# bababyVN/medical-image-segmentation-and-classification

Measured on AMD Instinct MI355X. Metric: images/sec (train step) Attention U-Net 256x256 bs=32/GPU, higher is better.
Workload: dtype bf16; 1 GPU; AttentionUNet 256x256 train step (fwd+BCE+bwd+clip+AdamW), bs=32/GPU, NHWC bf16 activations, fp32 master weights; global_batch=32, parallelism=dp1, hip_graph=False, wgrad_side_stream=True, plan_replay=C (mi355_plan_run)

## Files before the change

include/mi355conv.h:

```cpp
#ifndef MI355CONV_H_
#define MI355CONV_H_

#include <stdint.h>

#ifdef __cplusplus
extern "C" {
#endif

typedef struct ihipStream_t* mi355_stream_t;

enum { MI355_F32 = 0, MI355_BF16 = 1, MI355_F16 = 2 };
enum { MI355_OK = 0, MI355_ERR_ARG = -1, MI355_ERR_UNSUPPORTED = -2, MI355_ERR_RUNTIME = -3 };

int mi355_version(void);
const char* mi355_last_error(void);


int mi355_pack_input_nchw(const float* x, void* y, int N, int C, int H, int W, int Cpad, int dtype,
                          mi355_stream_t s);
int mi355_pack_input_im2col3(const float* x, void* y, int N, int C, int H, int W, int dtype, mi355_stream_t s);
int mi355_unpack_output_nchw(const void* x, float* y, int N, int C, int H, int W, int ld, int dtype,
                             mi355_stream_t s);
int mi355_pack_nchw(const float* x, void* y, int N, int C, int H, int W, int ld, int dtype, mi355_stream_t s);

int mi355_pack_conv_weight(const float* w, void* wf, void* wb, int Co, int Ci, int Cip, int KH, int KW,
                           int transposed, int dtype, mi355_stream_t s);

int mi355_pack_conv_weights_batched(const int64_t* table, int n, int fields ,
                                    int dtype, mi355_stream_t s);

int mi355_conv2d_igemm(const void* in, const void* wk, const float* bias, void* out,
                       int N, int Hi, int Wi, int Ci, int ldi,
                       int Ho, int Wo, int Co, int ldo,
                       int KH, int KW, int mul, int kmul, int off, int div, int up,
                       int accumulate, float* stats, int dtype, mi355_stream_t s);
int mi355_conv2d_igemm_variant(int Hi, int Wi, int Ci, int Ho, int Wo, int Co, int KH, int KW, int mul, int kmul, int off,
                               int div, int up, int dtype);
int mi355_conv2d_igemm_variant_n(int N, int Hi, int Wi, int Ci, int Ho, int Wo, int Co, int KH, int KW, int mul, int kmul,
                                 int off, int div, int up, int dtype);
int mi355_conv2d_igemm_dma_tile(int N, int Ho, int Wo, int Ci, int Co);
int mi355_conv2d_igemm_generic_tile(int N, int Ho, int Wo, int Co);
int mi355_conv2d_igemm_stat_rows(int N, int Hi, int Wi, int Ci, int Ho, int Wo, int Co, int KH, int KW,
                                 int mul, int kmul, int off, int div, int up, int dtype);
int mi355_conv2d_igemm_pool2_ok(int N, int Hi, int Wi, int Ci, int Ho, int Wo, int Co, int KH, int KW,
                                int mul, int kmul, int off, int div, int up, int dtype);
const char* mi355_conv2d_igemm_kernel_name(int N, int Hi, int Wi, int Ci, int Ho, int Wo, int Co, int KH, int KW,
                                           int mul, int kmul, int off, int div, int up, int dtype);

int mi355_conv2d_wgrad_splits(int N, int Ho, int Wo, int Ci, int Co, int KH, int KW);
int mi355_conv2d_wgrad_variant(int N, int Ho, int Wo, int KH, int KW, int stride, int pad, int dtype);
const char* mi355_conv2d_wgrad_kernel_name(int N, int Ho, int Wo, int Ci, int Co, int KH, int KW, int stride, int pad, int dtype);
int mi355_conv2d_wgrad(const void* x, const void* dy, float* ws, int splits,
                       int N, int Hi, int Wi, int Ci, int ldx,
                       int Ho, int Wo, int Co, int ldy,
                       int KH, int KW, int stride, int pad, int up, int dtype, mi355_stream_t s);
int mi355_conv2d_wgrad_multi_ok(int N, int Ho, int Wo, int dtype);
int mi355_conv2d_wgrad_multi(const void* x0, const void* dy0, const void* x1, const void* dy1, const void* x2, const void* dy2,
                             const void* x3, const void* dy3, const void* x4, const void* dy4, const void* x5, const void* dy5,
                             int napp, float* ws, int splits, int N, int Hi, int Wi, int Ci, int ldx, int Ho, int Wo, int Co,
                             int ldy, int up, int dtype, mi355_stream_t s);
int mi355_conv2d_wgrad_reduce(const float* ws, int splits, float* dw, int Co, int Ci, int Ci_real,
                              int KH, int KW, int transposed, float beta, mi355_stream_t s);


int mi355_rowreduce_blocks(long long M);
int mi355_bn_stats(const void* x, float* partial, long long M, int C, int ld, int dtype, mi355_stream_t s);
int mi355_bn_finalize(const float* partial, int nblocks, long long M, int C, const float* gamma,
                      const float* beta, float* running_mean, float* running_var, int64_t* nbt,
                      float momentum, float eps, float* scale, float* shift, float* mean, float* invstd,
                      mi355_stream_t s);
int mi355_fold_rows(const float* partial, int rows, int rowlen, float* out, int nsplit, mi355_stream_t s);
int mi355_bn_fold_bias(const float* bias, const float* scale, const float* shift, float* out, int C, mi355_stream_t s);
int mi355_bn_eval_coeffs(const float* gamma, const float* beta, const float* running_mean,
                         const float* running_var, float eps, int C, float* scale, float* shift,
                         mi355_stream_t s);
int mi355_bn_act(const void* x, int ldx, const float* scale, const float* shift,
                 const void* x2, int ldx2, const float* scale2, const float* shift2,
                 const void* res, int ldr, void* y, int ldy, long long M, int C, int act, int dtype,
                 mi355_stream_t s);
int mi355_bn_act_pool2(const void* x, int ldx, const float* scale, const float* shift, void* y, int ldy, void* p, int ldp,
                       int N, int H, int W, int C, int act, int dtype, mi355_stream_t s);
int mi355_bn_act_windows(const void* x, int ldx, const float* scale, const float* shift, const void* res, int ldr, void* y, int ldy,
                         int N, int H, int W, int C, int act, int dtype, mi355_stream_t s);
int mi355_bn_bwd_reduce_rows(long long M);
int mi355_bn_bwd_reduce(const void* dy, int lddy, const void* y, int ldy, const void* x, int ldx,
                        const float* mean, const float* invstd, const float* mscale, const float* mshift,
                        float* partial, long long M, int C, int act, int dtype, mi355_stream_t s);
int mi355_bn_bwd_finalize(const float* partial, int nblocks, int C, float* sums, float* dgamma, float* dbeta,
                          float acc, mi355_stream_t s);
int mi355_bn_bwd_finalize_at(const float* partial, int nblocks, int nq, int q0, int q1, int C, float* sums, float* dgamma,
                             float* dbeta, float acc, mi355_stream_t s);
int mi355_bn_bwd_apply(const void* dy, int lddy, const void* y, int ldy, const void* x, int ldx,
                       const float* gamma, const float* mean, const float* invstd, const float* mscale,
                       const float* mshift, const float* sums, void* dx, int lddx, void* dres, int lddres,
                       void* dpost, int lddpost, int post_acc, float* dbias_partial,
                       long long M, int C, int act, int dtype, mi355_stream_t s);
int mi355_bn_bwd_apply_post4(const void* dy, int lddy, const void* y, int ldy, const void* x, int ldx,
                             const float* gamma, const float* mean, const float* invstd, const float* mscale,
                             const float* mshift, const float* sums, void* dx, int lddx, void* dpost, int lddpost,
                             int post_acc, const void* ex0, const void* ex1, const void* ex2, const void* ex3, int ldex,
                             long long M, int C, int act, int dtype, mi355_stream_t s);
int mi355_bn_bwd_pool2_ok(int H, int W, int C, int dtype);
int mi355_bn_bwd_reduce_pool2_rows(long long M);
int mi355_bn_bwd_reduce_pool2(const void* dy, int lddy, const void* dp, int lddp, const void* x, int ldx, const float* mean,
                              const float* invstd, const float* mscale, const float* mshift, float* partial,
                              int N, int H, int W, int C, int dtype, mi355_stream_t s);
int mi355_bn_bwd_apply_pool2(const void* dy, int lddy, const void* dp, int lddp, const void* x, int ldx, const float* gamma,
                             const float* mean, const float* invstd, const float* mscale, const float* mshift,
                             const float* sums, void* dx, int lddx, int N, int H, int W, int C, int dtype, mi355_stream_t s);
int mi355_colsum_finalize(const float* partial, int nblocks, int stride, int C, float* out, float acc,
                          mi355_stream_t s);
int mi355_colsum(const void* x, int ld, float* partial, long long M, int C, int dtype, mi355_stream_t s);

int mi355_maxpool_fwd(const void* x, int ldx, void* y, int ldy, int N, int H, int W, int C,
                      int k, int stride, int pad, int dtype, mi355_stream_t s);
int mi355_maxpool_bwd(const void* x, int ldx, const void* dy, int lddy, void* dx, int lddx,
                      int N, int H, int W, int C, int k, int stride, int pad, int accumulate, int dtype,
                      mi355_stream_t s);
int mi355_upsample2_bwd(const void* dy, int lddy, void* dx, int lddx, int N, int H, int W, int C,
                        int accumulate, int dtype, mi355_stream_t s);
int mi355_add(const void* a, int lda, const void* b, int ldb, void* y, int ldy, long long M, int C, int dtype,
              mi355_stream_t s);
int mi355_relu_fwd(const void* x, int ldx, void* y, int ldy, long long M, int C, int dtype, mi355_stream_t s);
int mi355_relu_bwd(const void* dy, int lddy, const void* y, int ldy, void* dx, int lddx, long long M, int C,
                   int dtype, mi355_stream_t s);

int mi355_rowdot_fwd(const void* x, int ldx, const float* w, const float* b, float* z, float* partial,
                     long long M, int C, int HW, int K, int dtype, mi355_stream_t s);
int mi355_rowdot_bwd(const float* dz, const void* x, int ldx, const float* w, void* dx, int lddx,
                     float* partial, long long M, int C, int relu_mask, int HW, int K, int accumulate, int dtype,
                     mi355_stream_t s);
int mi355_gate_mul_fwd(const void* x, int ldx, const float* z, const float* scale, const float* shift,
                       void* y, int ldy, long long M, int C, int dtype, mi355_stream_t s);
int mi355_gate_mul_bwd(const void* dy, int lddy, const void* x, int ldx, const float* z, const float* scale,
                       const float* shift, const float* mean, const float* invstd, void* dx, int lddx,
                       int accumulate, float* dzn, float* partial, long long M, int C, int dtype,
                       mi355_stream_t s);
int mi355_bn1_bwd_apply(const float* dzn, const float* z, const float* gamma, const float* mean,
                        const float* invstd, const float* sums, float* dz, long long M, mi355_stream_t s);
int mi355_gate_psi_fwd_ok(int C, int dtype);
int mi355_gate_psi_fwd(const void* g1, int ldg, const void* x1, int ldx, const float* scale_g, const float* shift_g,
                       const float* scale_x, const float* shift_x, const float* w, const float* b, float* z,
                       float* partial, long long M, int C, int dtype, mi355_stream_t s);
int mi355_gate_bn_bwd_reduce_rows(long long M);
int mi355_gate_bn_bwd_reduce(const float* dz, const void* g1, int ldg, const void* x1, int ldx, const float* scale_g,
                             const float* shift_g, const float* mean_g, const float* invstd_g, const float* scale_x,
                             const float* shift_x, const float* mean_x, const float* invstd_x, const float* w,
                             float* partial, long long M, int C, int dtype, mi355_stream_t s);
int mi355_gate_bn_bwd_apply(const float* dz, const void* g1, int ldg, const void* x1, int ldx, const float* scale_g,
                            const float* shift_g, const float* mean_g, const float* invstd_g, const float* scale_x,
                            const float* shift_x, const float* mean_x, const float* invstd_x, const float* w,
                            const float* gamma_g, const float* gamma_x, const float* sums_g, const float* sums_x,
                            void* dg1, int lddg, void* dx1, int lddx, long long M, int C, int dtype, mi355_stream_t s);

int mi355_global_pool_fwd(const void* x, int ldx, float* y, int32_t* argmax, int N, int HW, int C, int is_max,
                          int dtype, mi355_stream_t s);
int mi355_global_pool_bwd(const float* dy, const int32_t* argmax, void* dx, int lddx, int N, int HW, int C,
                          int is_max, int dtype, mi355_stream_t s);
int mi355_linear_fwd(const float* x, const float* w, const float* bias, float* y, int B, int I, int O, int relu,
                     mi355_stream_t s);
int mi355_linear_bwd(const float* x, const float* w, const float* y, const float* dy, float* dx, float* dw,
                     float* db, int B, int I, int O, int relu, float beta, float* scratch, mi355_stream_t s);
int mi355_linear_bwd_scratch(int B, int I, int O);
int mi355_dropout_fwd(const float* x, float* y, uint8_t* mask, long long n, float p, uint64_t seed,
                      const int32_t* counter, mi355_stream_t s);
int mi355_dropout_bwd(const float* dy, const uint8_t* mask, float* dx, long long n, float p, mi355_stream_t s);

int mi355_bce_logits(const float* z, const float* t, float* loss, float* dz, const float* gscale, long long n,
                     mi355_stream_t s);
int mi355_ce_smooth(const float* z, const int64_t* y, float* loss, float* dz, const float* gscale, int B,
                    int C, float smoothing, mi355_stream_t s);
int mi355_ce_mix(const float* z, const int64_t* ya, const int64_t* yb, const float* lam, const float* weight, float* loss,
                 float* dz, const float* gscale, int B, int C, float smoothing, mi355_stream_t s);
int mi355_seg_loss_rows(int B, long long per);
int mi355_seg_loss_fwd(const float* z, const float* t, int B, long long per, float bce_weight, float dice_weight,
                       float smooth, int per_sample, float* partial, float* state, float* loss, mi355_stream_t s);
int mi355_seg_loss_bwd(const float* z, const float* t, int B, long long per, float bce_weight, const float* state,
                       const float* gscale, float* dz, mi355_stream_t s);
int mi355_sdist_ws_ints(int B, int H, int W);
int mi355_signed_dist2(const float* target, int B, int H, int W, float thr, int32_t* ws, long long ws_ints,
                       int32_t* sd2, mi355_stream_t s);
int mi355_boundary_loss_rows(int B, long long per);
int mi355_boundary_loss_fwd(const float* z, const int32_t* sd2, int B, long long per, float weight, const float* base,
                            float* partial, float* loss, mi355_stream_t s);
int mi355_boundary_loss_bwd(const float* z, const int32_t* sd2, int B, long long per, float weight, const float* gscale,
                            int accumulate, float* dz, mi355_stream_t s);
int mi355_segsort_tile(void);
int mi355_segsort_ws_ints(int S, long long len);
int mi355_segsort_f32(const float* keys, int S, long long len, int32_t* ws, long long ws_ints, int32_t* perm,
                      mi355_stream_t s);
int mi355_lovasz_ws_ints(int S, long long len);
int mi355_lovasz_fwd(const float* z, const float* t, int S, long long len, float thr, float weight, const float* base,
                     int32_t* ws, long long ws_ints, float* coef, float* loss, mi355_stream_t s);
int mi355_lovasz_bwd(const float* coef, long long n, const float* gscale, int accumulate, float* dz, mi355_stream_t s);
int mi355_rank_ws_ints(int S, long long len);
// ... 121 lines not shown
```

medical-image-segmentation-and-classification_amd/csrc/conv_gemm256.hpp:

```cpp
#pragma once
#include "common.hpp"

struct Gemm256Cfg {
  static constexpr int BM = 256, BN = 128, BK = 64, NS = 3;
  static constexpr int A_BYTES = BM * BK * 2, B_BYTES = BN * BK * 2, STAGE = A_BYTES + B_BYTES;
  static constexpr int C_PITCH = BN * 2 + 16;
  static constexpr int LDS_BYTES = NS * STAGE;
  static_assert(BM * C_PITCH + 4 * 2 * BN * 4 <= LDS_BYTES, "the C tile and the statistics scratch go on top of the dead ring");
};

template <typename T>
__global__ __launch_bounds__(512, 2) void conv_gemm256_kernel(const ConvArgs a, const int mode) {
  static_assert(sizeof(T) == 2, "bf16 / fp16 only");
  typedef Gemm256Cfg Cfg;
  constexpr int BM = Cfg::BM, BN = Cfg::BN, BK = Cfg::BK, NS = Cfg::NS, EPC = 8;
  constexpr int A_BYTES = Cfg::A_BYTES, STAGE = Cfg::STAGE, C_PITCH = Cfg::C_PITCH;
  constexpr int A_IT = BM / 8 / 8, B_IT = BN / 8 / 8, PER_TILE = A_IT + B_IT;
  extern __shared__ __attribute__((aligned(16))) unsigned char lds[];

  const int tid = threadIdx.x, lane = tid & 63, wave = __builtin_amdgcn_readfirstlane(tid >> 6);
  const int l16 = lane & 15, c4 = lane >> 4;
  const int wm = wave >> 1, wn = wave & 1;
  const int taps = a.KH * a.KW;
  const int NCOL = mode == 1 ? taps * a.Co : a.Co;
  const int NT = NCOL / BN;
  const int bid = xcd_tile(blockIdx.x, gridDim.x);
  const int mt = bid / NT, nt = bid - mt * NT;
  const int m0 = mt * BM, n0 = nt * BN;
  const int ptap = mode == 1 ? n0 / a.Co : 0, co0 = mode == 1 ? n0 - ptap * a.Co : n0;
  const T* __restrict__ in = reinterpret_cast<const T*>(a.in);
  const T* __restrict__ wk = reinterpret_cast<const T*>(a.wk);
  auto fsw = [](int row) { return (row >> 1) & 7; };

  const int lrow = lane >> 3, slot = lane & 7;
  const T* a_src[A_IT];
#pragma unroll
  for (int i = 0; i < A_IT; ++i) {
    const int row = (wave + 8 * i) * 8 + lrow;
    const int m = m0 + row;
    long long pix;
    if (mode == 1) {
      pix = m;
    } else {
      const int n = m / a.HoWo, rem = m - n * a.HoWo;
      const int ho = rem / a.Wo, wo = rem - ho * a.Wo;
      pix = ((long long)n * a.Hi + ho * a.mul) * a.Wi + wo * a.mul;
    }
    a_src[i] = in + pix * a.ldi + (slot ^ fsw(row)) * EPC;
  }
  const T* b_src[B_IT];
#pragma unroll
  for (int i = 0; i < B_IT; ++i) {
    const int row = (wave + 8 * i) * 8 + lrow;
    b_src[i] = wk + ((size_t)(co0 + row) * taps + ptap) * a.Ci + (slot ^ fsw(row)) * EPC;
  }
  const unsigned lds0 = lds_addr(lds);
  const int KC = a.Ci / BK;
  const int KT = (mode == 1 ? 1 : taps) * KC;
  int i_tap = 0, i_c0 = 0, i_stage = 0;
  size_t i_aoff = 0, i_boff = 0;
  auto issue_piece = [&](int j) __attribute__((always_inline)) {
    const unsigned st = lds0 + i_stage * STAGE;
    if (j < A_IT) dma16(a_src[j] + i_aoff, st + (wave + 8 * j) * 1024);
    else dma16(b_src[j - A_IT] + i_boff, st + A_BYTES + (wave + 8 * (j - A_IT)) * 1024);
  };
  auto issue_advance = [&]() __attribute__((always_inline)) {
    i_c0 += BK;
    if (i_c0 == a.Ci) {
      i_c0 = 0;
      ++i_tap;
    }
    const int kh = i_tap / a.KW, kw = i_tap - kh * a.KW;
    i_aoff = (mode == 1 ? (size_t)0 : ((size_t)kh * a.Wi + kw) * a.ldi) + i_c0;
    i_boff = (mode == 1 ? (size_t)0 : (size_t)i_tap * a.Ci) + i_c0;
    i_stage = i_stage + 1 == NS ? 0 : i_stage + 1;
  };

  f32x4 acc[4][4];
#pragma unroll
  for (int cb = 0; cb < 4; ++cb)
#pragma unroll
    for (int pb = 0; pb < 4; ++pb) acc[cb][pb] = f32x4{0.f, 0.f, 0.f, 0.f};

  int fa_w[4], fa_p[4];
#pragma unroll
  for (int b = 0; b < 4; ++b) {
    const int rw = wn * 64 + b * 16 + l16, rp = wm * 64 + b * 16 + l16;
    fa_w[b] = A_BYTES + rw * 128 + fsw(rw) * 16;
    fa_p[b] = rp * 128 + fsw(rp) * 16;
  }
  auto frag = [&](const unsigned char* st, int base, int kh2) __attribute__((always_inline)) {
    return *reinterpret_cast<const bf16x8*>(st + (base ^ ((kh2 * 4 + c4) << 4)));
  };

  int issued = 0;
#pragma unroll
  for (int t = 0; t < NS - 1; ++t) {
    if (issued < KT) {
#pragma unroll
      for (int j = 0; j < PER_TILE; ++j) issue_piece(j);
      issue_advance();
      ++issued;
    }
  }

  int stage = 0;
  for (int kt = 0; kt < KT; ++kt) {
    if (kt + 1 < KT) wait_vmcnt<PER_TILE>(); else wait_vmcnt<0>();
    __builtin_amdgcn_s_barrier();
    const unsigned char* st = lds + stage * STAGE;
    const bool more = issued < KT;
    bf16x8 w0[4], p0[4], w1[4], p1[4];
#pragma unroll
    for (int b = 0; b < 4; ++b) {
      w0[b] = frag(st, fa_w[b], 0);
      p0[b] = frag(st, fa_p[b], 0);
    }
#pragma unroll
    for (int b = 0; b < 4; ++b) {
      w1[b] = frag(st, fa_w[b], 1);
      p1[b] = frag(st, fa_p[b], 1);
    }
#pragma unroll
    for (int cb = 0; cb < 4; ++cb) {
#pragma unroll
      for (int pb = 0; pb < 4; ++pb) acc[cb][pb] = mfma_16x16x32<T>(w0[cb], p0[pb], acc[cb][pb]);
      if (more) {
        issue_piece(cb);
      }
    }
#pragma unroll
    for (int cb = 0; cb < 4; ++cb) {
#pragma unroll
      for (int pb = 0; pb < 4; ++pb) acc[cb][pb] = mfma_16x16x32<T>(w1[cb], p1[pb], acc[cb][pb]);
      if (more && cb < PER_TILE - 4) issue_piece(4 + cb);
    }
    if (more) {
      issue_advance();
      ++issued;
    }
    stage = stage + 1 == NS ? 0 : stage + 1;
  }
  __syncthreads();

  T* __restrict__ out = reinterpret_cast<T*>(a.out);
  unsigned char* const cst = lds;
  float* const red = reinterpret_cast<float*>(lds + BM * C_PITCH);
  struct alignas(8) Pack4 { T v[4]; };
#pragma unroll
  for (int cb = 0; cb < 4; ++cb) {
    const int ch = wn * 64 + cb * 16 + 4 * c4;
    const f32x4 bias4 = a.bias ? *reinterpret_cast<const f32x4*>(a.bias + co0 + ch) : f32x4{0.f, 0.f, 0.f, 0.f};
    f32x4 sm = {0.f, 0.f, 0.f, 0.f}, sq = {0.f, 0.f, 0.f, 0.f};
#pragma unroll
    for (int pb = 0; pb < 4; ++pb) {
      const int row = wm * 64 + pb * 16 + l16;
      Pack4 pk;
#pragma unroll
      for (int r = 0; r < 4; ++r) {
        const float v = acc[cb][pb][r] + bias4[r];
        pk.v[r] = from_f32<T>(a.relu ? fmaxf(v, 0.f) : v);
        const float q = to_f32<T>(pk.v[r]);
        sm[r] += q;
        sq[r] += q * q;
      }
      *reinterpret_cast<Pack4*>(cst + row * C_PITCH + ch * 2) = pk;
    }
    if (a.stats) {
#pragma unroll
      for (int r = 0; r < 4; ++r) {
        const float s1 = row16_sum(sm[r]), s2 = row16_sum(sq[r]);
        if (l16 == 0) {
          red[(wm * 2 + 0) * BN + ch + r] = s1;
          red[(wm * 2 + 1) * BN + ch + r] = s2;
        }
      }
    }
  }
  __syncthreads();
  if (a.stats && tid < 2 * BN) {
    const int q = tid / BN, c = tid - q * BN;
    float v = 0.f;
#pragma unroll
    for (int w = 0; w < 4; ++w) v += red[(w * 2 + q) * BN + c];
    a.stats[((size_t)mt * 2 + q) * a.Co + n0 + c] = v;
  }
  constexpr int CPRC = BN / EPC;
  const int pdh = ptap / a.KW, pdw = ptap - pdh * a.KW;
  for (int id = tid; id < BM * CPRC; id += 512) {
    const int row = id / CPRC, c = id - row * CPRC;
    const int m = m0 + row;
    size_t opix;
    if (mode == 1) {
      const int hw = a.Hi * a.Wi;
      const int n = m / hw, rem = m - n * hw;
      const int h = rem / a.Wi, w = rem - h * a.Wi;
      opix = ((size_t)n * a.Ho + 2 * h + pdh) * a.Wo + 2 * w + pdw;
    } else {
      opix = (size_t)m;
    }
    T* p = out + opix * a.ldo + co0 + c * EPC;
    Vec16<T> v = *reinterpret_cast<const Vec16<T>*>(cst + row * C_PITCH + c * 16);
    if (a.accumulate) {
      const Vec16<T> o = ld16<T>(p);
#pragma unroll
      for (int e = 0; e < EPC; ++e) v.v[e] = from_f32<T>(to_f32<T>(v.v[e]) + to_f32<T>(o.v[e]));
    }
    st16<T>(p, v);
  }
}

static int gemm256_mode(const ConvShape& s) {
  if (s.up || s.off != 0 || s.KH != s.KW || s.Ci % 64 != 0 || s.Co % 128 != 0) return 0;
  const long long out_px = (long long)s.N * s.Ho * s.Wo, in_px = (long long)s.N * s.Hi * s.Wi;
  if (s.KH == 1 && s.div == 1 && (s.mul == 1 || s.mul == 2) && (long long)(s.Ho - 1) * s.mul < s.Hi && (long long)(s.Wo - 1) * s.mul < s.Wi)
    return out_px % 256 == 0 ? 1 : 0;
  if (s.KH == 2 && s.div == 1 && s.mul == 2 && s.kmul == 1 && 2 * s.Ho == s.Hi && 2 * s.Wo == s.Wi) return out_px % 256 == 0 ? 1 : 0;
  if (s.KH == 2 && s.div == 2 && s.mul == 1 && s.kmul == -1 && s.Ho == 2 * s.Hi && s.Wo == 2 * s.Wi) return in_px % 256 == 0 ? 2 : 0;
  return 0;
}
static long long gemm256_tiles(int mode, int N, int Hi, int Wi, int Ho, int Wo, int Co) {
  return mode == 2 ? (long long)N * Hi * Wi / 256 * (4 * Co / 128) : (long long)N * Ho * Wo / 256 * (Co / 128);
}

template <typename T>
static int launch_gemm256(const ConvArgs& a, int mode, hipStream_t s) {
  constexpr int lds_bytes = Gemm256Cfg::LDS_BYTES;
  static const hipError_t configured =
      hipFuncSetAttribute((const void*)conv_gemm256_kernel<T>, hipFuncAttributeMaxDynamicSharedMemorySize, lds_bytes);
  if (configured != hipSuccess)
    MI355_FAIL((int)configured, "conv_gemm256: cannot reserve %d B of LDS: %s", lds_bytes, hipGetErrorString(configured));
  const long long grid = gemm256_tiles(mode, a.N, a.Hi, a.Wi, a.Ho, a.Wo, a.Co);
  hipLaunchKernelGGL((conv_gemm256_kernel<T>), dim3((int)grid), dim3(512), lds_bytes, s, a, mode == 2 ? 1 : 0);
  MI355_LAUNCH_CHECK();
  return MI355_OK;
}
```

medical-image-segmentation-and-classification_amd/csrc/conv_igemm.hip:

```cpp
#include "common.hpp"
#include <stdlib.h>

struct ConvArgs {
  const void* in;
  const void* wk;
  const float* bias;
  void* out;
  int N, Hi, Wi, Ci, ldi;
  int Ho, Wo, Co, ldo;
  int KH, KW;
  int mul, kmul, off, dshift, up;
  int accumulate;
  int relu;
  int pool2;
  float* stats;
  int M;
  int HoWo;
  int Hlog, Wlog;
};

template <typename T> struct Frag;
template <> struct Frag<bf16_t> {
  static __device__ __forceinline__ void mma(const uint4& a, const uint4& b, f32x16& c) {
    c = __builtin_amdgcn_mfma_f32_32x32x16_bf16(__builtin_bit_cast(bf16x8, a), __builtin_bit_cast(bf16x8, b), c, 0,
// ... 323 lines not shown
  int ikh = 0, ikw = 0, ic0 = 0, issued = 0;
  auto advance = [&]() {
    ic0 += BK;
    if (ic0 == a.Ci) {
      ic0 = 0;
      if (++ikw == a.KW) {
        ikw = 0;
        ++ikh;
      }
    }
  };
#pragma unroll
  for (int s = 0; s < NS - 1; ++s) {
    if (issued < KT) {
      issue_tile(s, ikh, ikw, ic0);
      advance();
      ++issued;
    }
  }
  if (KT >= NS - 1) wait_vmcnt<(NS - 2) * PER_TILE>(); else wait_vmcnt<0>();
  __builtin_amdgcn_s_barrier();

  int stage = 0, istage = NS - 1;
  for (int kt = 0; kt < KT; ++kt) {
    const bool more = issued < KT;
    if (more) {
      issue_tile(istage, ikh, ikw, ic0);
      advance();
      ++issued;
      istage = (istage + 1 == NS) ? 0 : istage + 1;
    }
    const unsigned char* la = lds + stage * STAGE;
    const unsigned char* lb = la + A_BYTES;
#pragma unroll
    for (int kq = 0; kq < KQ; ++kq) {
      const int c = kq * 2 + h;
      uint4 af[MI], bf[NI];
#pragma unroll
      for (int mi = 0; mi < MI; ++mi) {
        const int row = wm * WTM + mi * 32 + r32;
        af[mi] = *reinterpret_cast<const uint4*>(la + row * P + swz(row, c));
      }
#pragma unroll
      for (int ni = 0; ni < NI; ++ni) {
        const int row = wn * WTN + ni * 32 + r32;
        bf[ni] = *reinterpret_cast<const uint4*>(lb + row * P + swz(row, c));
      }
#pragma unroll
      for (int mi = 0; mi < MI; ++mi)
#pragma unroll
        for (int ni = 0; ni < NI; ++ni) Frag<T>::mma(af[mi], bf[ni], acc[mi][ni]);
    }
    stage = (stage + 1 == NS) ? 0 : stage + 1;
    if (more) wait_vmcnt<(NS - 2) * PER_TILE>(); else wait_vmcnt<0>();
    __builtin_amdgcn_s_barrier();
  }

  T* __restrict__ out = reinterpret_cast<T*>(a.out);
  float bcol[NI];
#pragma unroll
  for (int ni = 0; ni < NI; ++ni) bcol[ni] = a.bias ? a.bias[n0 + wn * WTN + ni * 32 + r32] : 0.f;
  float* const red = reinterpret_cast<float*>(lds + C_BYTES);
  static_assert(LDS_BYTES >= C_BYTES + WM * 2 * BN * 4, "no room for the statistics scratch");
  if (a.stats) {
#pragma unroll
    for (int ni = 0; ni < NI; ++ni) {
      float sm = 0.f, sq = 0.f;
#pragma unroll
      for (int mi = 0; mi < MI; ++mi)
#pragma unroll
        for (int r = 0; r < 16; ++r) {
          const int row = wm * WTM + mi * 32 + (r & 3) + 8 * (r >> 2) + 4 * h;
          const float v = (m0 + row < a.M) ? to_f32<T>(from_f32<T>(a.relu ? fmaxf(acc[mi][ni][r] + bcol[ni], 0.f) : acc[mi][ni][r] + bcol[ni])) : 0.f;
          sm += v;
          sq += v * v;
        }
      sm += __shfl_xor(sm, 32, 64);
      sq += __shfl_xor(sq, 32, 64);
      if (h == 0) {
        red[(wm * 2 + 0) * BN + wn * WTN + ni * 32 + r32] = sm;
        red[(wm * 2 + 1) * BN + wn * WTN + ni * 32 + r32] = sq;
      }
    }
  }
#pragma unroll
  for (int mi = 0; mi < MI; ++mi)
#pragma unroll
    for (int ni = 0; ni < NI; ++ni)
#pragma unroll
      for (int r = 0; r < 16; ++r) {
        const int row = wm * WTM + mi * 32 + (r & 3) + 8 * (r >> 2) + 4 * h;
        const int col = wn * WTN + ni * 32 + r32;
        *reinterpret_cast<T*>(lds + row * C_PITCH + col * 2) = from_f32<T>(a.relu ? fmaxf(acc[mi][ni][r] + bcol[ni], 0.f) : acc[mi][ni][r] + bcol[ni]);
      }
  __syncthreads();
  if (a.stats && tid < 2 * BN) {
    const int q = tid / BN, c = tid - q * BN;
    float v = 0.f;
#pragma unroll
    for (int w = 0; w < WM; ++w) v += red[(w * 2 + q) * BN + c];
    a.stats[((size_t)mt * 2 + q) * a.Co + n0 + c] = v;
  }
  constexpr int CPRC = BN / EPC;
  for (int id = tid; id < BM * CPRC; id += 256) {
    const int row = id / CPRC, c = id - row * CPRC;
    const int m = m0 + row;
    if (m < a.M) {
      T* p = out + (size_t)m * a.ldo + n0 + c * EPC;
      Vec16<T> v = *reinterpret_cast<const Vec16<T>*>(lds + row * C_PITCH + c * 16);
      if (a.accumulate) {
        const Vec16<T> o = ld16<T>(p);
#pragma unroll
        for (int e = 0; e < EPC; ++e) v.v[e] = from_f32<T>(to_f32<T>(v.v[e]) + to_f32<T>(o.v[e]));
      }
      st16<T>(p, v);
    }
  }
}

template <auto KERNEL, int BN>
static int launch_tiles(const ConvArgs& a, hipStream_t s) {
  hipLaunchKernelGGL(KERNEL, dim3(ceil_div(a.M, 128) * (a.Co / BN)), dim3(256), 0, s, a);
  MI355_LAUNCH_CHECK();
  return MI355_OK;
}
template <typename T, int BN, int BK, int NS>
static int launch_dma(const ConvArgs& a, hipStream_t s) { return launch_tiles<conv_igemm_dma_kernel<T, BN, BK, NS>, BN>(a, s); }

struct ConvShape { int N, Hi, Wi, Ci, Ho, Wo, Co, KH, KW, mul, kmul, off, div, up, dtype; };

#include "conv3x3_halo.hpp"
#include "conv3x3_halo_pp.hpp"
#include "conv3x3_halo_pp128.hpp"
#include "conv3x3_ws.hpp"
#include "conv1x1_stream.hpp"
#include "conv_gemm256.hpp"

template <typename T, int BK>
static int launch_bn(const ConvArgs& a, hipStream_t s, int bn) {
  switch (bn) {
    case 128: return launch_tiles<conv_igemm_kernel<T, 128, BK>, 128>(a, s);
    case 64: return launch_tiles<conv_igemm_kernel<T, 64, BK>, 64>(a, s);
    default: return launch_tiles<conv_igemm_kernel<T, 32, BK>, 32>(a, s);
  }
}

enum IgemmVariant { IG_GENERIC = 0, IG_DMA, IG_HALO_8x32, IG_HALO_16x16, IG_STREAM1x1, IG_HALO_PP, IG_HALO_PP128, IG_WS64, IG_WS128, IG_GEMM256 };

struct ConvChoice {
  IgemmVariant variant;
  IgemmVariant shape_variant;
  int bn, bk, ns;
  int gemm256;
  int stat_rows;
  bool pool2;
};

static int env_int(const char* name, int dflt) { return getenv(name) ? atoi(getenv(name)) : dflt; }
static int device_cus() {
  static const int cus = [] {
    int dev = 0, n = 0;
    if (hipGetDevice(&dev) != hipSuccess || hipDeviceGetAttribute(&n, hipDeviceAttributeMultiprocessorCount, dev) != hipSuccess || n <= 0) n = 256;
    return n;
  }();
  return cus;
}
struct Switches {
  int force_generic = getenv("MI355_IGEMM_VARIANT") ? atoi(getenv("MI355_IGEMM_VARIANT")) == 0 : 0;
  int halo_pp = env_int("MI355_HALO_PP", 0);
  int pp128 = env_int("MI355_HALO_PP128", 1), pp128_min_ci = env_int("MI355_HALO_PP128_MINCI", 256);
  int pp128_fill = env_int("MI355_PP128_FILL", 80);
  int ws64 = env_int("MI355_WS64", 1), ws128 = env_int("MI355_WS128", 1);
  long long ws_min_tiles = getenv("MI355_WS64_MIN_TILES") ? atoll(getenv("MI355_WS64_MIN_TILES")) : 4ll * device_cus();
  int ws128_tile_mult = env_int("MI355_WS128_TILE_MULT", 6);
  int gemm256 = env_int("MI355_GEMM256", 1);
  long long gemm256_min_tiles = getenv("MI355_GEMM256_MIN_TILES") ? atoll(getenv("MI355_GEMM256_MIN_TILES")) : 128;
  int dma_smallgrid = env_int("MI355_DMA_SMALLGRID", 1);
};
static const Switches& switches() { static const Switches sw{}; return sw; }

static bool halo_family(IgemmVariant v) {
  return v == IG_HALO_8x32 || v == IG_HALO_16x16 || v == IG_HALO_PP || v == IG_HALO_PP128 || v == IG_WS64 || v == IG_WS128;
}
static bool image_fits_descriptor(int Hi, int Wi, int ldi, int esz) { return (long long)Hi * Wi * ldi * esz < (1ll << 31); }

static int small_grid_tile_n(long long M, int Co, bool to32) {
  const long long rows = (M + 127) / 128;
  int bn = Co % 128 == 0 ? 128 : (Co % 64 == 0 ? 64 : 32);
  if (switches().dma_smallgrid) {
    const int cus = device_cus();
    if (bn == 128 && rows * (Co / 128) * 2 <= cus) bn = 64;
    if (bn == 64 && to32 && rows * (Co / 64) * 2 <= cus) bn = 32;
  }
  return bn;
}

static IgemmVariant shape_variant(const ConvShape& s, const Switches& sw) {
  if (!dtype_is_2byte(s.dtype) || sw.force_generic) return IG_GENERIC;
  const int Hlog = s.up ? 2 * s.Hi : s.Hi, Wlog = s.up ? 2 * s.Wi : s.Wi;
  const bool is3x3s1 = s.KH == 3 && s.KW == 3 && s.mul == 1 && s.div == 1 && s.Ho == Hlog && s.Wo == Wlog &&
                       ((s.kmul == 1 && s.off == -1) || (s.kmul == -1 && s.off == 1 && !s.up));
  if (is3x3s1 && s.Co % 64 == 0) {
    const bool t16x32 = s.Wo % 32 == 0 && s.Ho % 16 == 0;
    if (sw.halo_pp && t16x32) return IG_HALO_PP;
    if (sw.pp128 && s.Co % 128 == 0 && s.Ci % 64 == 0 && s.Ci >= sw.pp128_min_ci && t16x32) return IG_HALO_PP128;
    const int ws_rows = ws_tile_rows(s.Ci, s.Ho, s.Wo, s.Co);
    if (sw.ws64 && ws_rows == 8) return IG_WS64;
    if (sw.ws128 && ws_rows == 4) return IG_WS128;
    if (s.Wo % 32 == 0 && s.Ho % 8 == 0) return IG_HALO_8x32;
    if (s.Wo % 16 == 0 && s.Ho % 16 == 0) return IG_HALO_16x16;
  }
  if (s.KH == 1 && s.KW == 1 && s.mul == 1 && s.div == 1 && !s.up && s.off == 0 && s.Ho == s.Hi && s.Wo == s.Wi && stream1x1_shape(s.Ci, s.Co))
    return IG_STREAM1x1;
  ConvShape whole = s; whole.N = 256;
  if (sw.gemm256 && gemm256_mode(whole)) return IG_GEMM256;
  if (s.Co % 64 != 0 && s.Ci % 64 != 0) return IG_GENERIC;
  return IG_DMA;
}

static ConvChoice choose(const ConvShape& s) {
  const Switches& sw = switches();
  const int cus = device_cus(), N = s.N, Ho = s.Ho, Wo = s.Wo, Co = s.Co;
  const long long M = (long long)N * Ho * Wo;
  ConvChoice c = {};
  IgemmVariant v = c.shape_variant = shape_variant(s, sw);
  if (v == IG_WS64 || v == IG_WS128) {
    const long long S = (long long)N * (Ho / (v == IG_WS64 ? 8 : 4)) * (Wo / 32);
    if (!(S >= 8 && S * (Co / 64) >= sw.ws_min_tiles * (v == IG_WS128 ? sw.ws128_tile_mult : 1)))
      v = Ho % 8 == 0 ? IG_HALO_8x32 : (Ho % 16 == 0 && Wo % 16 == 0 ? IG_HALO_16x16 : IG_DMA);
  } else if (v == IG_HALO_PP128) {
    const long long grid = (long long)N * (Ho / 16) * (Wo / 32) * (Co / 128);
    const long long rounds = (grid + cus - 1) / cus;
    if (grid * 100 < rounds * cus * sw.pp128_fill) v = IG_HALO_8x32;
  } else if (v == IG_GEMM256) {
    c.gemm256 = gemm256_mode(s);
    if (!c.gemm256 || gemm256_tiles(c.gemm256, N, s.Hi, s.Wi, Ho, Wo, Co) < sw.gemm256_min_tiles) v = IG_DMA, c.gemm256 = 0;
  }
  if (halo_family(v) && !image_fits_descriptor(s.Hi, s.Wi, s.Ci, 2)) v = IG_DMA;
  c.variant = v; c.pool2 = halo_family(v);
  const bool k64 = s.Ci % 64 == 0;
  if (!dtype_is_2byte(s.dtype)) {
    c.bn = small_grid_tile_n(M, Co, true), c.bk = 16;
  } else if (v == IG_GENERIC) {
    c.bn = small_grid_tile_n(M, Co, true), c.bk = k64 ? 64 : 32;
  } else if (v == IG_DMA) {
    c.bn = small_grid_tile_n(M, Co, k64);
    c.bk = c.bn == 64 || (c.bn == 128 && !k64) ? 32 : 64;
    c.ns = c.bn == 128 && k64 ? 2 : 3;
  }
  switch (v) {
    case IG_HALO_PP:
    case IG_HALO_PP128: c.stat_rows = N * (Ho / 16) * (Wo / 32); break;
    case IG_WS128: c.stat_rows = ws_groups(N, Ho, Wo, Co, 4, cus); break;
    case IG_WS64: c.stat_rows = ws_groups(N, Ho, Wo, Co, 8, cus); break;
    case IG_HALO_8x32: c.stat_rows = N * (Ho / 8) * (Wo / 32); break;
    case IG_HALO_16x16: c.stat_rows = N * (Ho / 16) * (Wo / 16); break;
    case IG_DMA: c.stat_rows = ceil_div(M, 128); break;
    case IG_STREAM1x1: c.stat_rows = stream1x1_grid(M); break;
    case IG_GEMM256: c.stat_rows = c.gemm256 == 1 ? (int)(M / 256) : 0; break;
    default: break;
  }
  return c;
}

static ConvArgs conv_args(const ConvShape& s) {
  ConvArgs a = {};
  a.N = s.N; a.Hi = s.Hi; a.Wi = s.Wi; a.Ci = s.Ci;
  a.Ho = s.Ho; a.Wo = s.Wo; a.Co = s.Co;
  a.KH = s.KH; a.KW = s.KW; a.mul = s.mul; a.kmul = s.kmul; a.off = s.off;
  a.dshift = s.div == 1 ? 0 : (s.div == 2 ? 1 : 2); a.up = s.up ? 1 : 0;
  a.M = s.N * s.Ho * s.Wo; a.HoWo = s.Ho * s.Wo;
  a.Hlog = s.up ? 2 * s.Hi : s.Hi; a.Wlog = s.up ? 2 * s.Wi : s.Wi;
  return a;
}

enum { IG_NAME_LEN = 64 };
#define IG_KERNEL(LAUNCH, ...)            \
  if (!name) return LAUNCH;               \
  return snprintf(name, IG_NAME_LEN, __VA_ARGS__) < 0 ? MI355_ERR_ARG : MI355_OK
template <typename T>
static int launch_or_name(const ConvChoice& c, const ConvArgs& a, hipStream_t st, char* name) {
  if constexpr (sizeof(T) == 4) {
    IG_KERNEL((launch_bn<T, 16>(a, st, c.bn)), "conv_igemm_kernel<f32,%d,16>", c.bn);
  } else {
    switch (c.variant) {
      case IG_HALO_PP: IG_KERNEL(launch_halo_pp<T>(a, st), "conv3x3_halo_pp_kernel");
      case IG_HALO_PP128: IG_KERNEL(launch_halo_pp128<T>(a, st), "conv3x3_halo_pp128_kernel");
      case IG_WS64: IG_KERNEL((launch_ws<T, 64, 8>(a, st, device_cus())), "conv3x3_ws_kernel<64,8>");
      case IG_WS128: IG_KERNEL((launch_ws<T, 128, 4>(a, st, device_cus())), "conv3x3_ws_kernel<128,4>");
      case IG_HALO_8x32: IG_KERNEL((launch_halo_rw<T, 8, 32>(a, st)), "conv3x3_halo_rw_kernel<8,32>");
      case IG_HALO_16x16: IG_KERNEL((launch_halo_rw<T, 16, 16>(a, st)), "conv3x3_halo_rw_kernel<16,16>");
      case IG_STREAM1x1: IG_KERNEL(launch_stream1x1<T>(a, st), "conv1x1_stream_kernel<%d,%d>", a.Ci, a.Co);
      case IG_GEMM256: IG_KERNEL(launch_gemm256<T>(a, c.gemm256, st), "conv_gemm256_kernel");
      case IG_DMA:
        switch (c.bn * 100 + c.bk) {
          case 12864: IG_KERNEL((launch_dma<T, 128, 64, 2>(a, st)), "conv_igemm_dma_kernel<128,64,2>");
          case 12832: IG_KERNEL((launch_dma<T, 128, 32, 3>(a, st)), "conv_igemm_dma_kernel<128,32,3>");
          case 6432: IG_KERNEL((launch_dma<T, 64, 32, 3>(a, st)), "conv_igemm_dma_kernel<64,32,3>");
          default: IG_KERNEL((launch_dma<T, 32, 64, 3>(a, st)), "conv_igemm_dma_kernel<32,64,3>");
        }
      default:
        IG_KERNEL((c.bk == 64 ? launch_bn<T, 64>(a, st, c.bn) : launch_bn<T, 32>(a, st, c.bn)), "conv_igemm_kernel<bf16,%d,%d>", c.bn, c.bk);
    }
  }
}
#undef IG_KERNEL

#define GEOM_PARAMS int Hi, int Wi, int Ci, int Ho, int Wo, int Co, int KH, int KW, int mul, int kmul, int off, int div, int up, int dtype
#define GEOM_SHAPE(N) ConvShape{N, Hi, Wi, Ci, Ho, Wo, Co, KH, KW, mul, kmul, off, div, up, dtype}
extern "C" int mi355_conv2d_igemm_variant(GEOM_PARAMS) { return (int)choose(GEOM_SHAPE(1)).shape_variant; }
extern "C" int mi355_conv2d_igemm_variant_n(int N, GEOM_PARAMS) { return (int)choose(GEOM_SHAPE(N)).variant; }
extern "C" int mi355_conv2d_igemm_stat_rows(int N, GEOM_PARAMS) { return choose(GEOM_SHAPE(N)).stat_rows; }
extern "C" int mi355_conv2d_igemm_pool2_ok(int N, GEOM_PARAMS) { return choose(GEOM_SHAPE(N)).pool2; }
extern "C" int mi355_conv2d_igemm_dma_tile(int N, int Ho, int Wo, int Ci, int Co) { return small_grid_tile_n((long long)N * Ho * Wo, Co, Ci % 64 == 0); }
extern "C" int mi355_conv2d_igemm_generic_tile(int N, int Ho, int Wo, int Co) { return small_grid_tile_n((long long)N * Ho * Wo, Co, true); }
extern "C" const char* mi355_conv2d_igemm_kernel_name(int N, GEOM_PARAMS) {
  static thread_local char name[IG_NAME_LEN];
  const ConvShape s = GEOM_SHAPE(N); const ConvChoice c = choose(s);
  const int rc = dispatch_dtype(dtype, "conv2d_igemm_kernel_name", [&](auto tag) { return launch_or_name<decltype(tag)>(c, conv_args(s), nullptr, name); });
  return rc == MI355_OK ? name : nullptr;
}

extern "C" int mi355_conv2d_igemm(const void* in, const void* wk, const float* bias, void* out, int N, int Hi, int Wi,
                                  int Ci, int ldi, int Ho, int Wo, int Co, int ldo, int KH, int KW, int mul, int kmul,
                                  int off, int div, int up, int accumulate, float* stats, int dtype, mi355_stream_t s) {
  MI355_CHECK_ARG(in && wk && out, "conv2d_igemm: null pointer");
  MI355_CHECK_ARG(N > 0 && Hi > 0 && Wi > 0 && Ho > 0 && Wo > 0 && KH > 0 && KW > 0, "conv2d_igemm: bad extent");
  MI355_CHECK_ARG(div == 1 || div == 2 || div == 4, "conv2d_igemm: div must be 1, 2 or 4 (got %d)", div);
  MI355_CHECK_ARG(Co % 32 == 0, "conv2d_igemm: Co=%d must be a multiple of 32", Co);
  MI355_CHECK_ARG(ldi >= Ci && ldo >= Co, "conv2d_igemm: channel stride smaller than channel count");
  MI355_CHECK_ARG((long long)N * Ho * Wo < (1ll << 31) && (long long)N * Hi * Wi < (1ll << 31),
                  "conv2d_igemm: pixel count overflows int32");
  MI355_CHECK_ARG(dtype == MI355_BF16 || dtype == MI355_F16 || dtype == MI355_F32, "conv2d_igemm: unknown dtype %d", dtype);
  const int esz = dtype_is_2byte(dtype) ? 2 : 4;
  MI355_CHECK_ARG(((uintptr_t)in % 16) == 0 && ((uintptr_t)wk % 16) == 0 && ((uintptr_t)out % 16) == 0 &&
                      (ldi * esz) % 16 == 0 && (ldo * esz) % 16 == 0,
                  "conv2d_igemm: pointers / channel strides must be 16-byte aligned");
  MI355_CHECK_ARG(Ci % (esz == 2 ? 32 : 16) == 0, "conv2d_igemm: Ci=%d must be a multiple of %d", Ci, esz == 2 ? 32 : 16);
  const ConvShape shape = GEOM_SHAPE(N);
  const ConvChoice c = choose(shape);
  MI355_CHECK_ARG(!halo_family(c.variant) || image_fits_descriptor(Hi, Wi, ldi, esz),
                  "conv2d_igemm: an image of %d x %d pixels at a channel stride of %d is 2 GiB or more: beyond the 32-bit lane offsets of "
                  "the halo kernels' buffer descriptors", Hi, Wi, ldi);
  MI355_CHECK_ARG(!stats || (c.stat_rows > 0 && !(accumulate & 1)),
                  "conv2d_igemm: fused statistics are not available for this shape/dtype (mi355_conv2d_igemm_stat_rows == 0)");
  ConvArgs a = conv_args(shape);
  a.in = in; a.wk = wk; a.bias = bias; a.out = out;
  a.ldi = ldi; a.ldo = ldo;
  a.accumulate = accumulate & 1;
  a.relu = (accumulate >> 1) & 1;
  a.pool2 = (accumulate >> 2) & 1;
  MI355_CHECK_ARG(!a.pool2 || (c.pool2 && !stats),
                  "conv2d_igemm: the 2x2-sum epilogue exists for the halo kernel only (mi355_conv2d_igemm_variant >= 2)");
  a.stats = stats;
  return dispatch_dtype(dtype, "conv2d_igemm", [&](auto tag) { return launch_or_name<decltype(tag)>(c, a, (hipStream_t)s, nullptr); });
}
```

Measured before the change: 2160 images/s.

## Add narrow-N small-K config for gemm256 conv used by 1x1 mode-1 shapes

Templates the gemm256 conv kernel on a config (wave layout, columns per wave, pipeline stages, waves per EU, fixed mode) and adds a BN=64, two-stage variant for mode-1 1x1 convolutions with Ci up to 512. The smaller tile halves accumulator and LDS footprint so more workgroups fit per CU and the grid doubles, which targets low occupancy and poor latency hiding on short-K GEMMs. The DMA issue schedule and wait counts are generalised to match. It risks more redundant A-tile loads, because each A tile is now reused across half as many output columns.

```diff
diff --git a/include/mi355conv.h b/include/mi355conv.h
--- a/include/mi355conv.h
+++ b/include/mi355conv.h
@@ -41,6 +41,8 @@
 int mi355_conv2d_igemm_dma_tile(int N, int Ho, int Wo, int Ci, int Co);
 int mi355_conv2d_igemm_generic_tile(int N, int Ho, int Wo, int Co);
 int mi355_conv2d_igemm_stat_rows(int N, int Hi, int Wi, int Ci, int Ho, int Wo, int Co, int KH, int KW,
+                                 int mul, int kmul, int off, int div, int up, int dtype);
+int mi355_conv2d_igemm_gemm_tile(int N, int Hi, int Wi, int Ci, int Ho, int Wo, int Co, int KH, int KW,
                                  int mul, int kmul, int off, int div, int up, int dtype);
 int mi355_conv2d_igemm_pool2_ok(int N, int Hi, int Wi, int Ci, int Ho, int Wo, int Co, int KH, int KW,
                                 int mul, int kmul, int off, int div, int up, int dtype);
diff --git a/medical-image-segmentation-and-classification_amd/csrc/conv_gemm256.hpp b/medical-image-segmentation-and-classification_amd/csrc/conv_gemm256.hpp
--- a/medical-image-segmentation-and-classification_amd/csrc/conv_gemm256.hpp
+++ b/medical-image-segmentation-and-classification_amd/csrc/conv_gemm256.hpp
@@ -1,26 +1,34 @@
 #pragma once
 #include "common.hpp"
 
-struct Gemm256Cfg {
-  static constexpr int BM = 256, BN = 128, BK = 64, NS = 3;
+template <int WN_, int CBW_, int NS_, int WAVES_PER_EU_, bool MODE0_>
+struct GemmCfg {
+  static constexpr int WN = WN_, CBW = CBW_;
+  static constexpr int BM = 256, BN = WN * CBW * 16, BK = 64, NS = NS_, WAVES = 4 * WN, THREADS = 64 * WAVES;
+  static constexpr int WAVES_PER_EU = WAVES_PER_EU_;
+  static constexpr bool MODE0 = MODE0_;
   static constexpr int A_BYTES = BM * BK * 2, B_BYTES = BN * BK * 2, STAGE = A_BYTES + B_BYTES;
   static constexpr int C_PITCH = BN * 2 + 16;
   static constexpr int LDS_BYTES = NS * STAGE;
+  static_assert(WAVES == 8 && BN % 64 == 0, "eight waves share the DMA pieces: 8 rows x 128 B each");
   static_assert(BM * C_PITCH + 4 * 2 * BN * 4 <= LDS_BYTES, "the C tile and the statistics scratch go on top of the dead ring");
 };
-
-template <typename T>
-__global__ __launch_bounds__(512, 2) void conv_gemm256_kernel(const ConvArgs a, const int mode) {
+typedef GemmCfg<2, 4, 3, 2, false> Gemm256Cfg;
+typedef GemmCfg<2, 2, 2, 4, true> GemmSmallKCfg;
+static_assert(2 * GemmSmallKCfg::LDS_BYTES <= 160 * 1024, "two small-K workgroups per CU");
+
+template <typename T, typename Cfg = Gemm256Cfg>
+__global__ __launch_bounds__(512, Cfg::WAVES_PER_EU) void conv_gemm256_kernel(const ConvArgs a, const int mode_arg) {
   static_assert(sizeof(T) == 2, "bf16 / fp16 only");
-  typedef Gemm256Cfg Cfg;
-  constexpr int BM = Cfg::BM, BN = Cfg::BN, BK = Cfg::BK, NS = Cfg::NS, EPC = 8;
+  constexpr int BM = Cfg::BM, BN = Cfg::BN, BK = Cfg::BK, NS = Cfg::NS, EPC = 8, WN = Cfg::WN, CBW = Cfg::CBW;
   constexpr int A_BYTES = Cfg::A_BYTES, STAGE = Cfg::STAGE, C_PITCH = Cfg::C_PITCH;
   constexpr int A_IT = BM / 8 / 8, B_IT = BN / 8 / 8, PER_TILE = A_IT + B_IT;
+  const int mode = Cfg::MODE0 ? 0 : mode_arg;
   extern __shared__ __attribute__((aligned(16))) unsigned char lds[];
 
   const int tid = threadIdx.x, lane = tid & 63, wave = __builtin_amdgcn_readfirstlane(tid >> 6);
   const int l16 = lane & 15, c4 = lane >> 4;
-  const int wm = wave >> 1, wn = wave & 1;
+  const int wm = wave / WN, wn = wave % WN;
   const int taps = a.KH * a.KW;
   const int NCOL = mode == 1 ? taps * a.Co : a.Co;
   const int NT = NCOL / BN;
@@ -76,17 +84,17 @@
     i_stage = i_stage + 1 == NS ? 0 : i_stage + 1;
   };
 
-  f32x4 acc[4][4];
-#pragma unroll
-  for (int cb = 0; cb < 4; ++cb)
+  f32x4 acc[CBW][4];
+#pragma unroll
+  for (int cb = 0; cb < CBW; ++cb)
 #pragma unroll
     for (int pb = 0; pb < 4; ++pb) acc[cb][pb] = f32x4{0.f, 0.f, 0.f, 0.f};
 
-  int fa_w[4], fa_p[4];
+  int fa_w[CBW], fa_p[4];
 #pragma unroll
   for (int b = 0; b < 4; ++b) {
-    const int rw = wn * 64 + b * 16 + l16, rp = wm * 64 + b * 16 + l16;
-    fa_w[b] = A_BYTES + rw * 128 + fsw(rw) * 16;
+    const int rw = wn * (CBW * 16) + b * 16 + l16, rp = wm * 64 + b * 16 + l16;
+    if (b < CBW) fa_w[b] = A_BYTES + rw * 128 + fsw(rw) * 16;
     fa_p[b] = rp * 128 + fsw(rp) * 16;
   }
   auto frag = [&](const unsigned char* st, int base, int kh2) __attribute__((always_inline)) {
@@ -106,34 +114,35 @@
 
   int stage = 0;
   for (int kt = 0; kt < KT; ++kt) {
-    if (kt + 1 < KT) wait_vmcnt<PER_TILE>(); else wait_vmcnt<0>();
+    if (NS > 2 && kt + 1 < KT) wait_vmcnt<(NS - 2) * PER_TILE>(); else wait_vmcnt<0>();
     __builtin_amdgcn_s_barrier();
     const unsigned char* st = lds + stage * STAGE;
     const bool more = issued < KT;
-    bf16x8 w0[4], p0[4], w1[4], p1[4];
+    bf16x8 w0[CBW], p0[4], w1[CBW], p1[4];
 #pragma unroll
     for (int b = 0; b < 4; ++b) {
-      w0[b] = frag(st, fa_w[b], 0);
+      if (b < CBW) w0[b] = frag(st, fa_w[b], 0);
       p0[b] = frag(st, fa_p[b], 0);
     }
 #pragma unroll
     for (int b = 0; b < 4; ++b) {
-      w1[b] = frag(st, fa_w[b], 1);
+      if (b < CBW) w1[b] = frag(st, fa_w[b], 1);
       p1[b] = frag(st, fa_p[b], 1);
     }
 #pragma unroll
-    for (int cb = 0; cb < 4; ++cb) {
+    for (int cb = 0; cb < CBW; ++cb) {
 #pragma unroll
       for (int pb = 0; pb < 4; ++pb) acc[cb][pb] = mfma_16x16x32<T>(w0[cb], p0[pb], acc[cb][pb]);
       if (more) {
-        issue_piece(cb);
+        if (cb < PER_TILE) issue_piece(cb);
+        if (cb + 2 * CBW < PER_TILE) issue_piece(cb + 2 * CBW);
       }
     }
 #pragma unroll
-    for (int cb = 0; cb < 4; ++cb) {
+    for (int cb = 0; cb < CBW; ++cb) {
 #pragma unroll
       for (int pb = 0; pb < 4; ++pb) acc[cb][pb] = mfma_16x16x32<T>(w1[cb], p1[pb], acc[cb][pb]);
-      if (more && cb < PER_TILE - 4) issue_piece(4 + cb);
+      if (more && CBW + cb < PER_TILE) issue_piece(CBW + cb);
     }
     if (more) {
       issue_advance();
@@ -148,8 +157,8 @@
   float* const red = reinterpret_cast<float*>(lds + BM * C_PITCH);
   struct alignas(8) Pack4 { T v[4]; };
 #pragma unroll
-  for (int cb = 0; cb < 4; ++cb) {
-    const int ch = wn * 64 + cb * 16 + 4 * c4;
+  for (int cb = 0; cb < CBW; ++cb) {
+    const int ch = wn * (CBW * 16) + cb * 16 + 4 * c4;
     const f32x4 bias4 = a.bias ? *reinterpret_cast<const f32x4*>(a.bias + co0 + ch) : f32x4{0.f, 0.f, 0.f, 0.f};
     f32x4 sm = {0.f, 0.f, 0.f, 0.f}, sq = {0.f, 0.f, 0.f, 0.f};
 #pragma unroll
@@ -223,15 +232,24 @@
   return mode == 2 ? (long long)N * Hi * Wi / 256 * (4 * Co / 128) : (long long)N * Ho * Wo / 256 * (Co / 128);
 }
 
-template <typename T>
-static int launch_gemm256(const ConvArgs& a, int mode, hipStream_t s) {
-  constexpr int lds_bytes = Gemm256Cfg::LDS_BYTES;
+static int gemm256_tile_n(int mode, const ConvShape& s, int max_ci) {
+  return mode == 1 && s.KH == 1 && s.mul == 1 && s.Ci <= max_ci ? GemmSmallKCfg::BN : Gemm256Cfg::BN;
+}
+
+template <typename T, typename Cfg>
+static int launch_gemm256_cfg(const ConvArgs& a, int mode, long long grid, hipStream_t s) {
+  constexpr int lds_bytes = Cfg::LDS_BYTES;
   static const hipError_t configured =
-      hipFuncSetAttribute((const void*)conv_gemm256_kernel<T>, hipFuncAttributeMaxDynamicSharedMemorySize, lds_bytes);
+      hipFuncSetAttribute((const void*)conv_gemm256_kernel<T, Cfg>, hipFuncAttributeMaxDynamicSharedMemorySize, lds_bytes);
   if (configured != hipSuccess)
     MI355_FAIL((int)configured, "conv_gemm256: cannot reserve %d B of LDS: %s", lds_bytes, hipGetErrorString(configured));
-  const long long grid = gemm256_tiles(mode, a.N, a.Hi, a.Wi, a.Ho, a.Wo, a.Co);
-  hipLaunchKernelGGL((conv_gemm256_kernel<T>), dim3((int)grid), dim3(512), lds_bytes, s, a, mode == 2 ? 1 : 0);
+  hipLaunchKernelGGL((conv_gemm256_kernel<T, Cfg>), dim3((int)grid), dim3(Cfg::THREADS), lds_bytes, s, a, mode == 2 ? 1 : 0);
   MI355_LAUNCH_CHECK();
   return MI355_OK;
 }
+template <typename T>
+static int launch_gemm256(const ConvArgs& a, int mode, int bn, hipStream_t s) {
+  const long long tiles = gemm256_tiles(mode, a.N, a.Hi, a.Wi, a.Ho, a.Wo, a.Co);
+  if (bn == GemmSmallKCfg::BN) return launch_gemm256_cfg<T, GemmSmallKCfg>(a, mode, tiles * (Gemm256Cfg::BN / GemmSmallKCfg::BN), s);
+  return launch_gemm256_cfg<T, Gemm256Cfg>(a, mode, tiles, s);
+}
diff --git a/medical-image-segmentation-and-classification_amd/csrc/conv_igemm.hip b/medical-image-segmentation-and-classification_amd/csrc/conv_igemm.hip
--- a/medical-image-segmentation-and-classification_amd/csrc/conv_igemm.hip
+++ b/medical-image-segmentation-and-classification_amd/csrc/conv_igemm.hip
@@ -499,6 +499,7 @@
   IgemmVariant shape_variant;
   int bn, bk, ns;
   int gemm256;
+  int gemm_bn;
   int stat_rows;
   bool pool2;
 };
@@ -522,6 +523,7 @@
   int ws128_tile_mult = env_int("MI355_WS128_TILE_MULT", 6);
   int gemm256 = env_int("MI355_GEMM256", 1);
   long long gemm256_min_tiles = getenv("MI355_GEMM256_MIN_TILES") ? atoll(getenv("MI355_GEMM256_MIN_TILES")) : 128;
+  int gemm_smallk_max_ci = env_int("MI355_GEMM_SMALLK", 1) ? env_int("MI355_GEMM_SMALLK_MAXCI", 512) : 0;
   int dma_smallgrid = env_int("MI355_DMA_SMALLGRID", 1);
 };
 static const Switches& switches() { static const Switches sw{}; return sw; }
@@ -582,6 +584,7 @@
   } else if (v == IG_GEMM256) {
     c.gemm256 = gemm256_mode(s);
     if (!c.gemm256 || gemm256_tiles(c.gemm256, N, s.Hi, s.Wi, Ho, Wo, Co) < sw.gemm256_min_tiles) v = IG_DMA, c.gemm256 = 0;
+    else c.gemm_bn = gemm256_tile_n(c.gemm256, s, sw.gemm_smallk_max_ci);
   }
   if (halo_family(v) && !image_fits_descriptor(s.Hi, s.Wi, s.Ci, 2)) v = IG_DMA;
   c.variant = v; c.pool2 = halo_family(v);
@@ -638,7 +641,7 @@
       case IG_HALO_8x32: IG_KERNEL((launch_halo_rw<T, 8, 32>(a, st)), "conv3x3_halo_rw_kernel<8,32>");
       case IG_HALO_16x16: IG_KERNEL((launch_halo_rw<T, 16, 16>(a, st)), "conv3x3_halo_rw_kernel<16,16>");
       case IG_STREAM1x1: IG_KERNEL(launch_stream1x1<T>(a, st), "conv1x1_stream_kernel<%d,%d>", a.Ci, a.Co);
-      case IG_GEMM256: IG_KERNEL(launch_gemm256<T>(a, c.gemm256, st), "conv_gemm256_kernel");
+      case IG_GEMM256: IG_KERNEL(launch_gemm256<T>(a, c.gemm256, c.gemm_bn, st), "conv_gemm256_kernel");
       case IG_DMA:
         switch (c.bn * 100 + c.bk) {
           case 12864: IG_KERNEL((launch_dma<T, 128, 64, 2>(a, st)), "conv_igemm_dma_kernel<128,64,2>");
@@ -661,6 +664,7 @@
 extern "C" int mi355_conv2d_igemm_pool2_ok(int N, GEOM_PARAMS) { return choose(GEOM_SHAPE(N)).pool2; }
 extern "C" int mi355_conv2d_igemm_dma_tile(int N, int Ho, int Wo, int Ci, int Co) { return small_grid_tile_n((long long)N * Ho * Wo, Co, Ci % 64 == 0); }
 extern "C" int mi355_conv2d_igemm_generic_tile(int N, int Ho, int Wo, int Co) { return small_grid_tile_n((long long)N * Ho * Wo, Co, true); }
+extern "C" int mi355_conv2d_igemm_gemm_tile(int N, GEOM_PARAMS) { return choose(GEOM_SHAPE(N)).gemm_bn; }
 extern "C" const char* mi355_conv2d_igemm_kernel_name(int N, GEOM_PARAMS) {
   static thread_local char name[IG_NAME_LEN];
   const ConvShape s = GEOM_SHAPE(N); const ConvChoice c = choose(s);
```

Result: no change. 2171 images/s (median of 6 runs) (+0.5%).
